# HKUST-Aerial-Robotics/DenseSurfelMapping

Hardware: AMD Instinct MI355X
Metric: depth frames fused/sec @ KITTI 1226x370 (higher is better)
Workload: dtype f32

## Files before the change

densesurfelmapping_amd/csrc/dsm_k_superpixel.h:

```cpp
#pragma once
#include "dsm_k_common.h"

namespace dsm {

constexpr int kInitLanes = 16, kInitSeedsPerBlock = 256 / kInitLanes;
template <bool BATCH> __global__ __launch_bounds__(256) void k_init_seeds(const DeviceCtx ctx, const DeviceCtx *__restrict__ batch) {
    const BlockOf blk = block_of<BATCH>();
    DeviceCtx batch_ctx;
    if (BATCH) batch_ctx = load_ctx(batch + blk.z);
    const DeviceCtx *__restrict__ c = BATCH ? &batch_ctx : &ctx;
    const int tid = threadIdx.x, lane = lane_id();
    const int r = tid & (kInitLanes - 1);
    const int s = blk.x * kInitSeedsPerBlock + tid / kInitLanes;
    if (blk.x == 0 && tid < kSweeps * kWorkers) c->first_empty[tid] = kIntMax;
    if (blk.x == 0 && tid == 0) c->work_count[0] = c->fit_big_count[0] = 0;
    if (blk.x == 0 && tid < 2 * kSweeps) c->rest_count[tid] = 0;
    const FrameParams &fp = c->params[(unsigned)(c->cursor[0] * c->cursor_mul + c->cursor_add) % (unsigned)c->n_params];
    const uint8_t *img = c->img_base + (int64_t)fp.slot * c->slot_elems;
    const float *dep = c->depth_base + (int64_t)fp.slot * c->slot_elems;
    if (blk.x == 0 && tid < 64) {
        FrameCur *wc = c->cur;
        const int t = tid;
        if (t < 16) wc->p.pose[t] = fp.pose[t];
        else if (t < 32) wc->p.inv[t - 16] = fp.inv[t - 16];
        else if (t == 32) { wc->p.ref_idx = fp.ref_idx; wc->p.slot = fp.slot; }
        else if (t == 33) wc->img = img;
        else if (t == 34) wc->dep = dep;
    }
    const int w = c->w, h = c->h, pitch = c->pitch;
    const bool live = s < c->n_seed;
    const int sc = live ? s : 0;
    const int gx = sc % c->gw, gy = sc / c->gw;
    int ix = gx * kCell + kCell / 2, iy = gy * kCell + kCell / 2;
    if (ix > w - 1) ix = w - 1;
    if (iy > h - 1) iy = h - 1;
    const int wx0 = gx * kCell + kCell / 2 - kCell, wy0 = gy * kCell + kCell / 2 - kCell;
    const int x_lo = wx0 < 0 ? 0 : wx0, x_hi = wx0 + 2 * kCell > w - 1 ? w - 1 : wx0 + 2 * kCell;
    const int y_lo = wy0 < 0 ? 0 : wy0, y_hi = wy0 + 2 * kCell > h - 1 ? h - 1 : wy0 + 2 * kCell;
    const int y = wy0 + r;
    const bool row_in = y >= y_lo && y < y_hi;
    float md = dep[iy * pitch + ix];
    const float mi = (float)img[iy * pitch + ix];
    float4 v[4];
#pragma unroll
    for (int q = 0; q < 4; q++) {
        const int x = wx0 + 4 * q;
        v[q] = (row_in && x >= 0) ? *reinterpret_cast<const float4 *>(dep + y * pitch + x) : make_float4(0, 0, 0, 0);
    }
    bool hit = false;
    float first = 0.0f;
#pragma unroll
    for (int q = 3; q >= 0; q--) {
        const float e[4] = {v[q].x, v[q].y, v[q].z, v[q].w};
#pragma unroll
        for (int t = 3; t >= 0; t--) {
            const int x = wx0 + 4 * q + t;
            if (row_in && x >= x_lo && x < x_hi && e[t] > flt_below(0.01)) { hit = true; first = e[t]; }
        }
    }
    const unsigned long long m = __ballot(hit);
    const unsigned rows = (unsigned)(m >> (lane & ~(kInitLanes - 1))) & 0xffffu;
    const int src = (lane & ~(kInitLanes - 1)) + (rows ? __ffs((int)rows) - 1 : 0);
    const float scanned = __shfl(first, src);
    if (md < flt_above(0.01) && rows) md = scanned;
    if (!live || r != 0) return;
    c->core[s] = make_float4((float)ix, (float)iy, mi, md);
    c->inv_depth[s] = 1.0 / (double)md;
    c->tmin[s] = -1;
}

template <bool BATCH> __global__ __launch_bounds__(256) void k_init_seeds_lanes(const DeviceCtx ctx, const DeviceCtx *__restrict__ batch) {
    const BlockOf blk = block_of<BATCH>();
    DeviceCtx batch_ctx;
    if (BATCH) batch_ctx = load_ctx(batch + blk.z);
    const DeviceCtx *__restrict__ c = BATCH ? &batch_ctx : &ctx;
    const int tid = threadIdx.x;
    const int s = blk.x * 256 + tid;
    if (blk.x == 0 && tid < kSweeps * kWorkers) c->first_empty[tid] = kIntMax;
    if (blk.x == 0 && tid == 0) c->work_count[0] = c->fit_big_count[0] = 0;
    if (blk.x == 0 && tid < 2 * kSweeps) c->rest_count[tid] = 0;
    const FrameParams &fp = c->params[(unsigned)(c->cursor[0] * c->cursor_mul + c->cursor_add) % (unsigned)c->n_params];
    const uint8_t *img = c->img_base + (int64_t)fp.slot * c->slot_elems;
    const float *dep = c->depth_base + (int64_t)fp.slot * c->slot_elems;
    if (blk.x == 0 && tid < 64) {
        FrameCur *wc = c->cur;
        const int t = tid;
        if (t < 16) wc->p.pose[t] = fp.pose[t];
        else if (t < 32) wc->p.inv[t - 16] = fp.inv[t - 16];
        else if (t == 32) { wc->p.ref_idx = fp.ref_idx; wc->p.slot = fp.slot; }
        else if (t == 33) wc->img = img;
        else if (t == 34) wc->dep = dep;
    }
    const int w = c->w, h = c->h, pitch = c->pitch;
    const bool live = s < c->n_seed;
    const int sc = live ? s : 0;
    int gx, gy;
    seed_cell(c, sc, gx, gy);
    int ix = gx * kCell + kCell / 2, iy = gy * kCell + kCell / 2;
    if (ix > w - 1) ix = w - 1;
    if (iy > h - 1) iy = h - 1;
    float md = dep[iy * pitch + ix];
    const float mi = (float)img[iy * pitch + ix];
    const bool need = live && md < flt_above(0.01);
    if (__ballot(need) != 0) {
        const int wx0 = gx * kCell + kCell / 2 - kCell, wy0 = gy * kCell + kCell / 2 - kCell;
        const int x_lo = wx0 < 0 ? 0 : wx0, x_hi = wx0 + 2 * kCell > w - 1 ? w - 1 : wx0 + 2 * kCell;
        const int y_lo = wy0 < 0 ? 0 : wy0, y_hi = wy0 + 2 * kCell > h - 1 ? h - 1 : wy0 + 2 * kCell;
        bool pending = need;
#pragma unroll 1
        for (int r0 = 0; r0 < 2 * kCell && __ballot(pending) != 0; r0 += 2) {
            float4 v[2][4];
            bool row_in[2];
#pragma unroll
            for (int k = 0; k < 2; k++) {
                const int y = wy0 + r0 + k;
                row_in[k] = pending && y >= y_lo && y < y_hi;
#pragma unroll
                for (int q = 0; q < 4; q++) {
                    const int x = wx0 + 4 * q;
                    v[k][q] = (row_in[k] && x >= 0) ? *reinterpret_cast<const float4 *>(dep + y * pitch + x) : make_float4(0, 0, 0, 0);
                }
            }
#pragma unroll
            for (int k = 0; k < 2; k++) {
                bool hit = false;
                float first = 0.0f;
#pragma unroll
                for (int q = 3; q >= 0; q--) {
                    const float e[4] = {v[k][q].x, v[k][q].y, v[k][q].z, v[k][q].w};
#pragma unroll
                    for (int t = 3; t >= 0; t--) {
                        const int x = wx0 + 4 * q + t;
                        if (row_in[k] && x >= x_lo && x < x_hi && e[t] > flt_below(0.01)) { hit = true; first = e[t]; }
                    }
                }
                if (pending && hit) { md = first; pending = false; }
            }
        }
    }
    if (!live) return;
    c->core[s] = make_float4((float)ix, (float)iy, mi, md);
    c->inv_depth[s] = 1.0 / (double)md;
    c->tmin[s] = -1;
}

constexpr int kTileW = 64, kTileCellsX = kTileW / kCell + 2;
template <int COLS> struct AssignTile {
    static constexpr int kH = 4 * COLS, kCellsY = (kH + kCell - 1) / kCell + 2;
};

constexpr int kResolveHeld = 8;
__device__ void resolve_worklist(const DeviceCtx *c, label_t *label) {
    const int n = c->work_count[0];
    if (n == 0) return;
    const int tid = threadIdx.x;
    int p[kResolveHeld], l[kResolveHeld], pk[kResolveHeld];
    bool ev[kResolveHeld];
#pragma unroll
    for (int k = 0; k < kResolveHeld; k++) p[k] = tid + k * 256 < n ? c->worklist[tid + k * 256] : -1;
#pragma unroll
    for (int k = 0; k < kResolveHeld; k++) {
        l[k] = p[k] >= 0 ? (int)label[p[k]] : 0;
        pk[k] = p[k] >= 0 ? (int)c->cand[p[k]] : 0;
    }
    for (;;) {
        int changed = 0;
        int tl[kResolveHeld], tp[kResolveHeld];
#pragma unroll
        for (int k = 0; k < kResolveHeld; k++) {
            if (k * 256 >= n) break;
            tl[k] = load_coherent(&c->tmin[l[k]]);
            tp[k] = load_coherent(&c->tmin[pk[k]]);
        }
#pragma unroll
        for (int k = 0; k < kResolveHeld; k++) {
            ev[k] = k * 256 < n && p[k] >= 0 && tl[k] < p[k];
            if (ev[k] && tp[k] > p[k]) {
                atomicMin(&c->tmin[pk[k]], p[k]);
                changed = 1;
            }
        }
        for (int i = tid + kResolveHeld * 256; i < n; i += 256) {
            const int q = c->worklist[i];
            const int lq = label[q], pq = c->cand[q];
            if (load_coherent(&c->tmin[lq]) < q && load_coherent(&c->tmin[pq]) > q) {
                atomicMin(&c->tmin[pq], q);
                changed = 1;
            }
        }
        if (!__syncthreads_or(changed)) break;
    }
#pragma unroll
    for (int k = 0; k < kResolveHeld; k++)
        if (ev[k]) label[p[k]] = (label_t)pk[k];
    for (int i = tid + kResolveHeld * 256; i < n; i += 256) {
        const int q = c->worklist[i];
        const int lq = label[q];
        if (load_coherent(&c->tmin[lq]) < q) label[q] = c->cand[q];
    }
}

template <bool FIRST, bool BATCH, int COLS> __global__ __launch_bounds__(256) void k_assign(const DeviceCtx ctx, const DeviceCtx *__restrict__ batch, int sweep) {
    constexpr int kColumn = COLS, kTileH = AssignTile<COLS>::kH, kTileCellsY = AssignTile<COLS>::kCellsY;
    const BlockOf blk = block_of<BATCH>();
    DeviceCtx batch_ctx;
    if (BATCH) batch_ctx = load_ctx(batch + blk.z);
    const DeviceCtx *__restrict__ c = BATCH ? &batch_ctx : &ctx;
    constexpr int kCells = kTileCellsX * kTileCellsY;
    __shared__ float4 s_core[kCells];
    __shared__ double s_inv[kCells];
    __shared__ float s_f[5][kCells];
    __shared__ unsigned short s_open[kTileW * kTileH];
    __shared__ int s_n_open;
    const FrameParams &fp = frame_params(c);
    const uint8_t *img = frame_image(c, fp);
    const float *dep = frame_depth(c, fp);
    const label_t *label_in = c->label;
    const int w = c->w, h = c->h, pitch = c->pitch, gw = c->gw, gh = c->gh;
    const int bx = blk.x * kTileW, by = blk.y * kTileH;
    const int cx0 = bx / kCell - 1, cy0 = by / kCell - 1;
    const int tid = threadIdx.x;
    if (tid == 0) s_n_open = 0;
    if (tid < kCells) {
        int gx = cx0 + tid % kTileCellsX, gy = cy0 + tid / kTileCellsX;
        gx = gx < 0 ? 0 : (gx > gw - 1 ? gw - 1 : gx);
        gy = gy < 0 ? 0 : (gy > gh - 1 ? gh - 1 : gy);
        const float4 v = c->core[gy * gw + gx];
        const double inv = c->inv_depth[gy * gw + gx];
        s_core[tid] = v;
        s_inv[tid] = inv;
        s_f[0][tid] = v.x * 0.25f;
        s_f[1][tid] = v.y * 0.25f;
        s_f[2][tid] = v.z;
        s_f[3][tid] = seed_s20(v.w, inv);
        s_f[4][tid] = v.w;
    }
    __syncthreads();
    auto settle = [&](int p, int l, int pick, int tl, int tp) {
        if (pick < 0) {
            atomicOr(c->status, kStatusBadPick);
            if (FIRST) label_put(c->label, (unsigned)p, 0);
        } else if (FIRST) {
            label_put(c->label, (unsigned)p, pick);
        } else if (tl == -1) {
            if (pick != l) label_put(c->label, (unsigned)p, pick);
            if (tp > p) atomicMin(&c->tmin[pick], p);
        } else if (pick != l) {
            label_put(c->cand, (unsigned)p, pick);
            const unsigned long long m = __ballot(true);
            const int rk = rank_below(m);
            int base = 0;
            if (rk == 0) base = atomicAdd(c->work_count, __popcll(m));
            base = __builtin_amdgcn_readlane(base, __ffsll((long long)m) - 1);
            c->worklist[base + rk] = p;
        }
    };
    auto tmin_of = [&](int s) {
        return __hip_atomic_load(reinterpret_cast<const int32_t *>(reinterpret_cast<const char *>(c->tmin) + ((unsigned)s << 2)), __ATOMIC_RELAXED,
                                 __HIP_MEMORY_SCOPE_AGENT);
    };
    const int x = bx + (tid & (kTileW - 1)), y0 = by + (tid / kTileW) * kColumn;
    if (x < w && y0 < h) {
        float pix_i[kColumn], pix_d[kColumn];
        int lab[kColumn], tl[kColumn], pick[kColumn];
        bool live[kColumn], sure[kColumn];
        const unsigned p0 = (unsigned)(__mul24(y0, pitch) + x);
#pragma unroll
        for (int r = 0; r < kColumn; r++) {
            const unsigned p = y0 + r < h ? p0 + (unsigned)(r * pitch) : p0, p4 = p << 2;
            pix_i[r] = (float)ld_off(img, p);
            pix_d[r] = ld_off(dep, p4);
            lab[r] = FIRST ? 0 : (int)ld_off(label_in, p << 1);
        }
        if (!FIRST) {
            const unsigned s_last = (unsigned)c->n_seed - 1u;
#pragma unroll
            for (int r = 0; r < kColumn; r++) tl[r] = ld_off(c->tmin, ((unsigned)lab[r] < s_last ? (unsigned)lab[r] : s_last) << 2);
        }
        const int li0 = __mul24(((y0 >> 3) - ((y0 & 7) < 4 ? 1 : 0)) - cy0, kTileCellsX) + (((x >> 3) - ((x & 7) < 4 ? 1 : 0)) - cx0);
        const PickCol quad = pick_col(x, y0, gw, gh, [&](int k, int, int, float &sx4, float &sy4, float &si, float &sd, float &s20) {
            const int li = li0 + (k >> 1) + (k & 1) * kTileCellsX;
            sx4 = s_f[0][li]; sy4 = s_f[1][li]; si = s_f[2][li]; s20 = s_f[3][li]; sd = s_f[4][li];
        });
#pragma unroll
        for (int r = 0; r < kColumn; r++) {
            const int y = y0 + r;
            live[r] = y < h && has_candidate_cell(x, y, gw, gh);
            const FastPick fpk = pick_seed_fast(quad, y, pix_i[r], pix_d[r], gw);
            pick[r] = fpk.seed;
            sure[r] = fpk.sure;
            if (FIRST && y < h && !live[r]) label_put(c->label, p0 + (unsigned)(r * pitch), -1);
        }
#pragma unroll
        for (int r = 0; r < kColumn; r++) {
            const bool open = live[r] && !sure[r];
            const unsigned long long m = __ballot(open);
            if (m) {
                const int rk = rank_below(m);
                int base = 0;
                if (open && rk == 0) base = atomicAdd(&s_n_open, __popcll(m));
                base = __builtin_amdgcn_readlane(base, __ffsll((long long)m) - 1);
                if (open) s_open[base + rk] = (unsigned short)((((tid / kTileW) * kColumn + r) << 6) | (tid & (kTileW - 1)));
            }
            live[r] = live[r] && !open;
        }
        int tp[kColumn];
        if (!FIRST) {
#pragma unroll
            for (int r = 0; r < kColumn; r++) tp[r] = tmin_of(live[r] ? pick[r] : 0);
        }
#pragma unroll
        for (int r = 0; r < kColumn; r++)
            if (live[r]) settle((int)p0 + r * pitch, lab[r], pick[r], FIRST ? 0 : tl[r], FIRST ? 0 : tp[r]);
    }
    __syncthreads();
    const int n_open = s_n_open;
    for (int i = tid; i < n_open; i += 256) {
        const unsigned e = s_open[i];
        const int ox = bx + (int)(e & 63u), oy = by + (int)(e >> 6);
        const unsigned p = (unsigned)(__mul24(oy, pitch) + ox);
        const float pi = (float)ld_off(img, p), pd = ld_off(dep, p << 2);
        const int l = FIRST ? 0 : label_at(label_in, p);
        const int pick = pick_seed(ox, oy, pi, pd, gw, gh, [&](int gx, int gy, float &sx, float &sy, float &si, bool &has_d, double &inv_d) {
            const int li = __mul24(gy - cy0, kTileCellsX) + (gx - cx0);
            const float4 v = s_core[li];
            sx = v.x; sy = v.y; si = v.z;
            has_d = v.w > 0;
            inv_d = s_inv[li];
        });
        settle((int)p, l, pick, FIRST ? 0 : ld_off(c->tmin, (unsigned)l << 2), FIRST || pick < 0 ? 0 : tmin_of(pick));
    }
}

template <bool BATCH> __global__ __launch_bounds__(256) void k_resolve(const DeviceCtx ctx, const DeviceCtx *__restrict__ batch, int sweep) {
    const BlockOf blk = block_of<BATCH>();
    DeviceCtx batch_ctx;
    if (BATCH) batch_ctx = load_ctx(batch + blk.z);
    const DeviceCtx *__restrict__ c = BATCH ? &batch_ctx : &ctx;
    resolve_worklist(c, c->label);
}

__device__ __forceinline__ float huber_ordered_sum(const float *lt, int nd, const unsigned long long tail[4],
                                                   const unsigned long long pos[4], double hr) {
    float a = 0.0f;
#pragma unroll
    for (int k = 0; k < 4; k++) {
        const int lim = nd - k * 64 < 64 ? nd - k * 64 : 64;
        if (lim <= 0) break;
        for (int j = 0; j < lim; j += kBlk) {
            const Blk16 v = load_blk(lt + k * 64 + j);
            const unsigned t16 = (unsigned)(tail[k] >> j) & 0xffffu, p16 = (unsigned)(pos[k] >> j) & 0xffffu;
            if (t16 == 0) {
#pragma unroll
                for (int q = 0; q < kBlk; q++) a += v.e[q];
            } else {
#pragma unroll
                for (int q = 0; q < kBlk; q++) {
                    const float a_core = a + v.e[q];
                    const float a_tail = (float)((double)a + (((p16 >> q) & 1u) ? hr : -1 * hr));
                    a = ((t16 >> q) & 1u) ? a_tail : a_core;
                }
            }
        }
    }
    return a;
}

__device__ __forceinline__ float huber_passes_wave(const float *dl, float *lt, int nd, float md, int it0, double hr, int lane) {
    const float hr_above = flt_above(hr);
    float dk[4];
#pragma unroll
    for (int k = 0; k < 4; k++) dk[k] = (k * 64 + lane < nd) ? dl[k * 64 + lane] : 0.0f;
    const int nk = (nd + 63) >> 6;
    for (int it = it0; it < 5; it++) {
        unsigned long long tail[4] = {0, 0, 0, 0}, pos[4] = {0, 0, 0, 0};
        int n_core = 0;
#pragma unroll
        for (int k = 0; k < 4; k++) {
            if (k >= nk) break;
            const int idx = k * 64 + lane;
            const bool valid = idx < nd;
            const float r = md - dk[k];
            const bool core = valid && fabsf(r) < hr_above;
            if (valid) lt[idx] = 2 * r;
            tail[k] = __ballot(valid && !core);
            pos[k] = __ballot(valid && !core && r > 0);
            n_core += __popcll(__ballot(core));
        }
        wave_lds_sync();
        const float a = huber_ordered_sum(lt, nd, tail, pos, hr);
        const float b = (float)(2 * n_core);
        const float delta = huber_newton_step(a, b);
        md = md + delta;
        wave_lds_sync();
        if (fabsf(delta) < flt_above(0.01)) break;
    }
    return md;
}

constexpr int kWin = 2 * kCell;

__device__ __forceinline__ void update_seed_finish(const DeviceCtx *__restrict__ c, int sweep, int s, int lane, int wx0, int wy0,
                                                   const float4 old, float *dl, float *lt, int cnt, int sdx, int sdy, int si, int nd) {
    stamp(c, sweep, s, 2, lane);
    const int cnt_si = wave_sum(si | (cnt << 16));
    cnt = cnt_si >> 16;
    si = cnt_si & 0xffff;
    if (cnt == 0) {
        if (lane == 0) atomicMin(&c->first_empty[sweep * kWorkers + chunk_of(c->n_seed, s)], s);
        return;
    }
    const int packed = wave_sum(sdx | (sdy << 16));
    const int sx = (packed & 0xffff) + cnt * wx0, sy = (packed >> 16) + cnt * wy0;
    wave_lds_sync();
    const float fn = (float)cnt;
    const float mi = (float)si / fn, mx = (float)sx / fn, my = (float)sy / fn;
    const float moved = fabsf(old.z - mi) + fabsf(old.x - mx) + fabsf(old.y - my);
    const int stable = moved < flt_above(0.2) ? 1 : 0;
    stamp(c, sweep, s, 3, lane);
    float md = 0.0f;
    wave_priority(nd);
    if (nd > 0) {
        pad_column(dl, nd, lane);
        pad_column(lt, nd, lane);
        wave_lds_sync();
        md = ordered_sum(dl, nd) / (float)nd;
        stamp(c, sweep, s, 4, lane);
        if (!mean_depth_is_settled(md)) md = huber_passes_wave(dl, lt, nd, md, 0, c->huber, lane);
    }
    stamp(c, sweep, s, 5, lane);
    if (kWaveStamps && c->stamps && lane == 0) c->stamps[((int64_t)sweep * c->n_seed + s) * 8 + 7] = nd;
    if (lane == 0) {
        c->core_stage[s] = make_float4(mx, my, mi, md);
        c->stable_stage[s] = stable;
    }
}

__device__ __forceinline__ void update_seed_wave(const DeviceCtx *__restrict__ c, int sweep, int s, float *dl, float *lt) {
    const int lane = lane_id();
    stamp(c, sweep, s, 0, lane);
    const FrameParams &fp = frame_params(c);
    const uint8_t *img = frame_image(c, fp);
    const float *dep = frame_depth(c, fp);
    const label_t *lbl = c->label;
    const int w = c->w, h = c->h, pitch = c->pitch;
    int gx, gy;
    seed_cell(c, s, gx, gy);
    const int wx0 = gx * kCell + kCell / 2 - kCell, wy0 = gy * kCell + kCell / 2 - kCell;
    const int t_self = c->tmin[s];
    if (t_self == kIntMax) return;
    const float4 old = c->core[s];
    stamp(c, sweep, s, 1, lane);
    int cnt = 0, sdx = 0, sdy = 0, si = 0, nd = 0;
    int lab[4], pi[4];
    float pd[4];
    bool pimg[4];
    const int x = wx0 + (lane & (kWin - 1)), y0 = wy0 + (lane >> 4);
    const bool x_in = x >= 0 && x < w;
    const int key0 = __mul24(y0, pitch) + x, row4 = 4 * pitch;
#pragma unroll
    for (int k = 0; k < 4; k++) {
        const int y = y0 + 4 * k;
        pimg[k] = x_in && y >= 0 && y < h;
        const int pk = pimg[k] ? key0 + k * row4 : 0;
        const unsigned o4 = (unsigned)pk << 2;
        lab[k] = (int)ld_off(lbl, (unsigned)pk << 1);
        pd[k] = ld_off(dep, o4);
        pi[k] = (int)ld_off(img, (unsigned)pk);
    }
#pragma unroll
    for (int k = 0; k < 4; k++) {
        const int idx = k * 64 + lane;
        const int y = y0 + 4 * k;
        const bool mem = pimg[k] && x < w - 1 && y < h - 1 && lab[k] == s;
        const float d = mem ? pd[k] : 0.0f;
        if (mem) {
            cnt += 1; sdx += idx & (kWin - 1); sdy += idx >> 4; si += pi[k];
        }
        const bool dv = mem && d > flt_below(0.1);
        const unsigned long long m = __ballot(dv);
        if (dv) dl[nd + rank_below(m)] = d;
        nd += __popcll(m);
    }
// ... 307 lines not shown
```

densesurfelmapping_amd/csrc/dsm_kernels.hip:

```cpp
#include "dsm_device.h"

#include "dsm_k_common.h"
#include "dsm_k_superpixel.h"
#include "dsm_k_planes.h"
#include "dsm_k_map.h"
#include "dsm_k_cloud.h"
#include "dsm_k_mesh.h"
#include "dsm_k_render.h"
#include "dsm_k_grid.h"
#include "dsm_k_field.h"
#include "dsm_k_carve.h"
#include "dsm_k_align.h"

namespace dsm {

const char *const kStageNames[kNumStages] = {
    "init_seeds", "assign_0",  "update_seeds_0", "commit_seeds_0", "assign_1",    "resolve_1",    "update_seeds_1", "commit_seeds_1",
    "assign_2",   "resolve_2", "update_seeds_2", "commit_seeds_2", "seed_points", "seed_fit", "fuse_surfels", "frame_tail",
};

template <bool E33>
static hipError_t launch_frame_as(const DeviceCtx &hc, int map_upper_bound, int tail_map_bound, bool with_compaction,
                                  hipStream_t st, hipEvent_t *ev, int stage_lo, int stage_hi, const DeviceCtx *d_batch, int n_batch, int lanes_from) {
    int stage = 0;
    hipError_t err = hipSuccess;
    const bool batched = d_batch != nullptr;
    const unsigned nz = batched ? (unsigned)n_batch : 1u;
#define hipLaunchStage(kernel_single, kernel_batch, grid, block, ...)                                        \
    do {                                                                                                     \
        if (stage - 1 >= stage_lo && stage - 1 <= stage_hi) {                                                \
            const dim3 g_((grid).x, (grid).y, nz);                                                           \
            if (batched) hipLaunchKernelGGL(kernel_batch, g_, block, 0, st, hc, d_batch, ##__VA_ARGS__);   \
            else hipLaunchKernelGGL(kernel_single, g_, block, 0, st, hc, d_batch, ##__VA_ARGS__);          \
        }                                                                                                    \
    } while (0)
#define DSM_MARK()                                                                      \
    do {                                                                                \
        if (ev) {                                                                       \
            err = hipEventRecord(ev[stage], st);                                        \
            if (err != hipSuccess) return err;                                          \
        }                                                                               \
        stage++;                                                                        \
    } while (0)
    const int S = hc.n_seed;
    const dim3 g_seed_thr((S + 255) / 256);
    const dim3 g_seed_wave((S + 3) / 4);
    const dim3 g_seed_lane((S + 63) / 64);
    const dim3 g_seed_rest((S + 63) / 64 + kRestOverBlocks);
    const bool lanes = batched && n_batch >= (lanes_from > 0 ? lanes_from : kLaneBatch);
    const dim3 g_tile1((hc.w + kTileW - 1) / kTileW, (hc.h + AssignTile<1>::kH - 1) / AssignTile<1>::kH);
    const dim3 g_tile4((hc.w + kTileW - 1) / kTileW, (hc.h + AssignTile<4>::kH - 1) / AssignTile<4>::kH);
    if (ev) hipLaunchKernelGGL(k_delay, dim3(1), dim3(64), 0, st, 40000LL);
    DSM_MARK();
    if (lanes) hipLaunchStage(k_init_seeds_lanes<true>, k_init_seeds_lanes<true>, g_seed_thr, dim3(256));
    else hipLaunchStage(k_init_seeds<false>, k_init_seeds<true>, dim3((S + kInitSeedsPerBlock - 1) / kInitSeedsPerBlock), dim3(256));
    DSM_MARK();
    for (int sweep = 0; sweep < kSweeps; sweep++) {
        if (sweep == 0) {
            if (lanes) hipLaunchStage((k_assign<true, true, 4>), (k_assign<true, true, 4>), g_tile4, dim3(256), sweep);
            else hipLaunchStage((k_assign<true, false, 1>), (k_assign<true, true, 1>), g_tile1, dim3(256), sweep);
            DSM_MARK();
        } else {
            if (lanes) hipLaunchStage((k_assign<false, true, 4>), (k_assign<false, true, 4>), g_tile4, dim3(256), sweep);
            else hipLaunchStage((k_assign<false, false, 1>), (k_assign<false, true, 1>), g_tile1, dim3(256), sweep);
            DSM_MARK();
            hipLaunchStage(k_resolve<false>, k_resolve<true>, dim3(1), dim3(256), sweep);
            DSM_MARK();
        }
        if (lanes) {
            hipLaunchStage(k_update_seeds<true>, k_update_seeds<true>, g_seed_lane, dim3(64), sweep);
            hipLaunchStage(k_update_seeds_rest<true>, k_update_seeds_rest<true>, g_seed_rest, dim3(64), sweep);
        } else {
            hipLaunchStage(k_update_seeds_wave<false>, k_update_seeds_wave<true>, g_seed_wave, dim3(256), sweep);
        }
        DSM_MARK();
        hipLaunchStage(k_commit_seeds<false>, k_commit_seeds<true>, g_seed_thr, dim3(256), sweep);
        DSM_MARK();
    }
    if (lanes) {
        hipLaunchStage(k_pixel_normals<true>, k_pixel_normals<true>, dim3((hc.w + 63) / 64, (hc.h + 4 * kNormalRows - 1) / (4 * kNormalRows)), dim3(256));
        hipLaunchStage(k_seed_stats<true>, k_seed_stats<true>, g_seed_lane, dim3(64));
    } else {
        hipLaunchStage(k_seed_points<false>, k_seed_points<true>, g_seed_wave, dim3(256));
    }
    DSM_MARK();
    const int fit_masks = lanes ? 1 : 0;
    hipLaunchStage((k_seed_fit<false, kFitAll>), (k_seed_fit<true, kFitSmall>), dim3((S + kFitSeeds - 1) / kFitSeeds), dim3(64), fit_masks);
    if (batched) hipLaunchStage((k_seed_fit<false, kFitAll>), (k_seed_fit<true, kFitLarge>), dim3(kFitLargeBlocks), dim3(64), fit_masks);
    hipLaunchStage((k_seed_finish<false, E33>), (k_seed_finish<true, E33>), g_seed_thr, dim3(256));
    DSM_MARK();
    int fuse_blocks = (map_upper_bound + 255) / 256;
    if (fuse_blocks < 1) fuse_blocks = 1;
    const int fuse_cap = batched ? resident_blocks(k_fuse_surfels<true, E33>, 256, kFuseBlocksPerCu) : resident_blocks(k_fuse_surfels<false, E33>, 256, kFuseBlocksPerCu);
    if (fuse_blocks > fuse_cap) fuse_blocks = fuse_cap;
    if (batched && nz > 1 && fuse_blocks > (fuse_cap / nz > 1 ? fuse_cap / nz : 1)) fuse_blocks = fuse_cap / nz > 1 ? fuse_cap / nz : 1;
    hipLaunchStage((k_fuse_surfels<false, E33>), (k_fuse_surfels<true, E33>), dim3(fuse_blocks), dim3(256));
    DSM_MARK();
    int tail_blocks = 1;
    if (with_compaction && tail_map_bound > kTailFastWords * 64) {
        tail_blocks = 1 + (tail_map_bound / 64 + kTailChunkWords) / kTailChunkWords;
        if (tail_blocks > kTailMaxBlocks) tail_blocks = kTailMaxBlocks;
    }
    hipLaunchStage(k_frame_tail<false>, k_frame_tail<true>, dim3(tail_blocks), dim3(1024), with_compaction ? 1 : 0);
    DSM_MARK();
    if (ev) {
        err = hipEventRecord(ev[stage], st);
        if (err != hipSuccess) return err;
    }
#undef DSM_MARK
#undef hipLaunchStage
    return hipGetLastError();
}

hipError_t launch_frame(const DeviceCtx &hc, bool eigen33, int map_upper_bound, int tail_map_bound, bool with_compaction,
                        hipStream_t st, hipEvent_t *ev, int stage_lo, int stage_hi, const DeviceCtx *d_batch, int n_batch, int lanes_from) {
    return eigen33 ? launch_frame_as<true>(hc, map_upper_bound, tail_map_bound, with_compaction, st, ev, stage_lo, stage_hi, d_batch, n_batch, lanes_from)
                   : launch_frame_as<false>(hc, map_upper_bound, tail_map_bound, with_compaction, st, ev, stage_lo, stage_hi, d_batch, n_batch, lanes_from);
}

}
```

densesurfelmapping_amd/csrc/dsm_math.h:

```cpp
#pragma once
#include <math.h>
#include <stdint.h>

#if defined(__HIPCC__) || defined(__HIP__)
#define DSM_HD __host__ __device__ __forceinline__
#else
#define DSM_HD static inline
#endif

namespace dsm {

constexpr int kCell = 8;
constexpr int kSweeps = 3;
constexpr int kWorkers = 10;
constexpr double kAngleCos = 0.1;

struct Intrinsics {
    float fx, fy, cx, cy;
};

DSM_HD constexpr float flt_below(double c) {
    const float f = (float)c;
    return (double)f <= c ? f : __builtin_bit_cast(float, __builtin_bit_cast(uint32_t, f) - 1u);
}
// ... 16 lines not shown
    float cost = 0.0f;
    cost += dist / (float)((kCell / 2) * (kCell / 2));
    float di = si - pix_i;
    cost = (float)((double)cost + div_by_100((double)(di * di)));
    no_d = cost;
    with_d = cost;
    if (seed_has_depth && pix_invd > 0) {
        float dd = (float)(seed_inv_depth - (double)pix_invd);
        with_d = (float)((double)cost + (double)(dd * dd) * 400.0);
        return true;
    }
    return false;
}

DSM_HD float pixel_inv_depth(float d) {
    float invd = 0.0f;
    if (d > flt_below(0.01)) invd = 1.0f / d;
    return invd;
}

DSM_HD bool has_candidate_cell(int x, int y, int gw, int gh) { return x < gw * kCell + kCell / 2 && y < gh * kCell + kCell / 2; }

template <typename LoadSeed>
DSM_HD int pick_seed(int x, int y, float pix_i, float pix_d, int gw, int gh, LoadSeed load) {
    const float invd = pixel_inv_depth(pix_d);
    const int bx = x / kCell, by = y / kCell;
    float best_d = 1e6f, best_n = 1e6f;
    int arg_d = -1, arg_n = -1;
    bool all_depth = true;
    const int xr = x % kCell, yr = y % kCell;
    const int gx0 = bx - (xr < kCell / 2 ? 1 : 0), gy0 = by - (yr < kCell / 2 ? 1 : 0);
    for (int jx = 0; jx < 2; jx++) {
        const int gx = gx0 + jx;
        if (!(gx >= 0 && gx < gw) || (jx == 1 && xr == kCell / 2)) continue;
        for (int jy = 0; jy < 2; jy++) {
            const int gy = gy0 + jy;
            if (!(gy >= 0 && gy < gh) || (jy == 1 && yr == kCell / 2)) continue;
            const int s = gy * gw + gx;
            float sx, sy, si;
            bool has_d;
            double inv_d;
            load(gx, gy, sx, sy, si, has_d, inv_d);
            float cn, cd;
            const bool with = pixel_cost(sx, sy, si, has_d, inv_d, pix_i, invd, x, y, cn, cd);
            all_depth = all_depth && with;
            if (cd < best_d) { best_d = cd; arg_d = s; }
            if (cn < best_n) { best_n = cn; arg_n = s; }
        }
    }
    return all_depth ? arg_d : arg_n;
}

struct FastCost {
    float c, err;
};
constexpr float kFastU = 5.9604645e-8f;

#if defined(__HIP_DEVICE_COMPILE__)
typedef float f32x2 __attribute__((ext_vector_type(2)));
DSM_HD f32x2 f2_make(float a, float b) { f32x2 r; r.x = a; r.y = b; return r; }
DSM_HD f32x2 f2_fma(f32x2 a, f32x2 b, f32x2 c) { return __builtin_elementwise_fma(a, b, c); }
DSM_HD f32x2 f2_mul(f32x2 a, f32x2 b) { return a * b; }
DSM_HD f32x2 f2_sub(f32x2 a, f32x2 b) { return a - b; }
DSM_HD float rcp_1ulp(float d) { return __builtin_amdgcn_rcpf(d); }
#else
struct f32x2 {
    float x, y;
};
DSM_HD f32x2 f2_make(float a, float b) { return f32x2{a, b}; }
DSM_HD f32x2 f2_fma(f32x2 a, f32x2 b, f32x2 c) { return f32x2{__builtin_fmaf(a.x, b.x, c.x), __builtin_fmaf(a.y, b.y, c.y)}; }
DSM_HD f32x2 f2_mul(f32x2 a, f32x2 b) { return f32x2{a.x * b.x, a.y * b.y}; }
DSM_HD f32x2 f2_sub(f32x2 a, f32x2 b) { return f32x2{a.x - b.x, a.y - b.y}; }
DSM_HD float rcp_1ulp(float d) {
    const float q = 1.0f / d;
    uint32_t b = __builtin_bit_cast(uint32_t, q);
    if ((b & 0x7f800000u) == 0u) return 0.0f;
    uint32_t hsh = __builtin_bit_cast(uint32_t, d) * 2654435761u;
    hsh ^= hsh >> 15;
    const uint32_t k = hsh % 3u;
    if (q == q && (b & 0x7f800000u) != 0x7f800000u) b += k == 1u ? 1u : (k == 2u ? 0xffffffffu : 0u);
    return __builtin_bit_cast(float, b);
}
#endif
DSM_HD f32x2 f2_splat(float a) { return f2_make(a, a); }

DSM_HD bool pixel_has_inv_depth(float d) { return d > flt_below(0.01) && d < __builtin_inff(); }
DSM_HD float pixel_p20(float d) { return 20.0f * rcp_1ulp(d); }
DSM_HD float seed_s20(float mean_depth, double inv_depth) { return mean_depth > 0 ? (float)(20.0 * inv_depth) : 0.0f; }

DSM_HD float fast_cost_df(float s20_abs_max) { return __builtin_fmaf(12.0f * kFastU, s20_abs_max, 2e-36f); }
DSM_HD float fast_cost_slack(float ad20, float df) {
    const float e2 = __builtin_fmaf(16.0f * kFastU, ad20, df);
    return e2 * __builtin_fmaf(2.0f, ad20, e2);
}
DSM_HD float fast_cost_err(float c, float slack) { return __builtin_fmaf(20.0f * kFastU, c, slack); }

DSM_HD FastCost pixel_cost_fast(float sx, float sy, float si, float s20, bool with_depth, float pix_i, float p20, int x, int y) {
    const float ddx = sx - (float)x;
    const float ax16 = (ddx * ddx) * 0.0625f;
    const float ddyq = sy * 0.25f - (float)y * 0.25f;
    const float dist16 = __builtin_fmaf(ddyq, ddyq, ax16);
    const float t = (si - pix_i) * 0.1f;
    const float c_no = __builtin_fmaf(t, t, dist16);
    const float dd20 = __builtin_fmaf(s20, with_depth ? 1.0f : 0.0f, with_depth ? -p20 : 0.0f);
    FastCost r;
    r.c = __builtin_fmaf(dd20, dd20, c_no);
    r.err = fast_cost_err(r.c, fast_cost_slack(fabsf(dd20), fast_cost_df(fabsf(s20))));
    return r;
}

struct PickCol {
    f32x2 ax16[2];
    f32x2 ax16_edge[2];
    f32x2 sy4[2], si[2], s20[2];
    bool depth_ok[2];
    float df;
    int base;
};
constexpr float kPickPenalty = 1e30f;
template <typename LoadSeedF> DSM_HD PickCol pick_col(int x, int y, int gw, int gh, LoadSeedF load) {
    PickCol q;
    const int xr = x & (kCell - 1), yr = y & (kCell - 1);
    const int gx0 = (x >> 3) - (xr < kCell / 2 ? 1 : 0), gy0 = (y >> 3) - (yr < kCell / 2 ? 1 : 0);
    static_assert(kCell == 8, "the shifts above");
    q.base = gy0 * gw + gx0;
    const bool col_ok[2] = {gx0 >= 0, gx0 + 1 < gw && xr != kCell / 2};
    const bool row_in[2] = {gy0 >= 0, gy0 + 1 < gh};
    float sx4[4], sy4[4], si[4], sd[4], s20[4];
    for (int k = 0; k < 4; k++) load(k, gx0 + (k >> 1), gy0 + (k & 1), sx4[k], sy4[k], si[k], sd[k], s20[k]);
    const f32x2 xq = f2_splat((float)x * 0.25f);
    for (int j = 0; j < 2; j++) {
        const f32x2 ddx4 = f2_sub(f2_make(sx4[2 * j], sx4[2 * j + 1]), xq);
        const f32x2 a = f2_mul(ddx4, ddx4);
        const bool in0 = col_ok[j] && row_in[0], in1 = col_ok[j] && row_in[1];
        q.ax16[j] = f2_make(in0 ? a.x : kPickPenalty, in1 ? a.y : kPickPenalty);
        q.ax16_edge[j] = f2_make(in0 ? a.x : kPickPenalty, kPickPenalty);
        q.sy4[j] = f2_make(sy4[2 * j], sy4[2 * j + 1]);
        q.si[j] = f2_make(si[2 * j], si[2 * j + 1]);
        q.s20[j] = f2_make(s20[2 * j], s20[2 * j + 1]);
    }
    q.df = fast_cost_df(fmaxf(fmaxf(fabsf(s20[0]), fabsf(s20[1])), fmaxf(fabsf(s20[2]), fabsf(s20[3]))));
    for (int j = 0; j < 2; j++)
        q.depth_ok[j] = !row_in[j] | ((!col_ok[0] | (sd[j] > 0)) & (!col_ok[1] | (sd[2 + j] > 0)));
    return q;
}
struct FastPickTrace {
    float err;
    bool all_depth;
};
struct FastPick {
    int seed;
    bool sure;
};
DSM_HD FastPick pick_seed_fast(const PickCol &q, int y, float pix_i, float pix_d, int gw, FastPickTrace *trace = nullptr) {
    const bool edge = (y & (kCell - 1)) == kCell / 2;
    const bool all_depth = pixel_has_inv_depth(pix_d) && q.depth_ok[0] && (q.depth_ok[1] || edge);
    const f32x2 mm = f2_splat(all_depth ? 1.0f : 0.0f), p20m = f2_splat(all_depth ? -pixel_p20(pix_d) : 0.0f);
    const f32x2 yq = f2_splat((float)y * 0.25f), pi = f2_splat(pix_i), tenth = f2_splat(0.1f);
    f32x2 c[2], dd20[2];
    for (int j = 0; j < 2; j++) {
        const f32x2 ddyq = f2_sub(q.sy4[j], yq);
        const f32x2 dist16 = f2_fma(ddyq, ddyq, edge ? q.ax16_edge[j] : q.ax16[j]);
        const f32x2 t = f2_mul(f2_sub(q.si[j], pi), tenth);
        const f32x2 c_no = f2_fma(t, t, dist16);
        dd20[j] = f2_fma(q.s20[j], mm, p20m);
        c[j] = f2_fma(dd20[j], dd20[j], c_no);
    }
    const float ck[4] = {c[0].x, c[0].y, c[1].x, c[1].y};
    const float ad_max = fmaxf(fmaxf(fabsf(dd20[0].x), fabsf(dd20[0].y)), fmaxf(fabsf(dd20[1].x), fabsf(dd20[1].y)));
    uint32_t key[4];
    for (int k = 0; k < 4; k++) key[k] = (__builtin_bit_cast(uint32_t, ck[k]) & ~3u) | (uint32_t)k;
    const uint32_t lo01 = key[0] < key[1] ? key[0] : key[1], hi01 = key[0] < key[1] ? key[1] : key[0];
    const uint32_t lo23 = key[2] < key[3] ? key[2] : key[3], hi23 = key[2] < key[3] ? key[3] : key[2];
    const uint32_t first = lo01 < lo23 ? lo01 : lo23;
    const uint32_t mid_a = lo01 < lo23 ? lo23 : lo01, mid_b = hi01 < hi23 ? hi01 : hi23;
    const uint32_t second = mid_a < mid_b ? mid_a : mid_b;
    const float c1 = __builtin_bit_cast(float, first), c2 = fminf(__builtin_bit_cast(float, second), 2e6f);
    const float err = fast_cost_err(c2, fast_cost_slack(ad_max, q.df));
    if (trace) { trace->err = err; trace->all_depth = all_depth; }
    FastPick r;
    r.seed = q.base + (int)(first & 1u) * gw + (int)((first >> 1) & 1u);
    r.sure = c1 + err < c2 - err && c1 + err < 1e6f;
    return r;
}
template <typename LoadSeedF>
DSM_HD FastPick pick_seed_fast(int x, int y, float pix_i, float pix_d, int gw, int gh, LoadSeedF load, FastPickTrace *trace = nullptr) {
    return pick_seed_fast(pick_col(x, y, gw, gh, load), y, pix_i, pix_d, gw, trace);
}

DSM_HD float huber_newton_step(float a, float b) { return (-a) / (b + 10.0f); }

DSM_HD bool mean_depth_is_settled(float md) { return md == __builtin_inff(); }

DSM_HD float huber_mean_depth(const float *list, int n, float sum, double huber) {
    const float hr_above = flt_above(huber);
    float md = sum / (float)n;
    if (mean_depth_is_settled(md)) return md;
    for (int it = 0; it < 5; it++) {
        float a = 0, b = 0;
        for (int k = 0; k < n; k++) {
            float r = md - list[k];
            if (fabsf(r) < hr_above) {
                a += 2 * r;
                b += 2;
            } else {
                a = (float)((double)a + (r > 0 ? huber : -1 * huber));
            }
        }
        float delta = huber_newton_step(a, b);
        md = md + delta;
        if (fabsf(delta) < flt_above(0.01)) break;
    }
    return md;
}

struct WindowPixel {
    bool member, has_depth, inlier;
};
DSM_HD WindowPixel window_pixel(bool row_in, bool col_in, bool label_is_seed, float d, float mean_depth, float hr_above) {
    WindowPixel p;
    p.member = row_in && col_in && label_is_seed;
    p.has_depth = p.member && d > flt_below(0.05);
    p.inlier = p.has_depth && fabsf(mean_depth - d) < hr_above;
    return p;
}

DSM_HD void back_project(const Intrinsics &k, float u, float v, float d, float &x, float &y, float &z) {
    x = (u - k.cx) / k.fx * d;
    y = (v - k.cy) / k.fy * d;
    z = d;
}

DSM_HD float ray_coeff(int u, float c, float f) { return ((float)u - c) / f; }

DSM_HD bool pixel_normal_rays(float rx0, float rx1, float ry0, float ry1, float d, float d_right, float d_down, float &nx, float &ny,
                              float &nz) {
    constexpr float kMin = flt_above(0.1);
    if (d < kMin || d_right < kMin || d_down < kMin) return false;
    const float px = rx0 * d, py = ry0 * d, pz = d;
    float rx = rx1 * d_right, ry = ry0 * d_right, rz = d_right;
    float dx = rx0 * d_down, dy = ry1 * d_down, dz = d_down;
    rx = rx - px; ry = ry - py; rz = rz - pz;
    dx = dx - px; dy = dy - py; dz = dz - pz;
    float ax = ry * dz - rz * dy, ay = rz * dx - rx * dz, az = rx * dy - ry * dx;
    float len = sqrtf(ax * ax + ay * ay + az * az);
    ax /= len; ay /= len; az /= len;
    float va = (ax * px + ay * py + az * pz) / sqrtf(px * px + py * py + pz * pz);
    if (fabsf(va) < flt_above(kAngleCos)) return false;
    nx = ax; ny = ay; nz = az;
    return true;
}

DSM_HD bool pixel_normal(const Intrinsics &k, int x, int y, float d, float d_right, float d_down, float &nx,
                         float &ny, float &nz) {
    constexpr float kMin = flt_above(0.1);
    if (d < kMin || d_right < kMin || d_down < kMin) return false;
    float px, py, pz, rx, ry, rz, dx, dy, dz;
    back_project(k, (float)x, (float)y, d, px, py, pz);
    back_project(k, (float)(x + 1), (float)y, d_right, rx, ry, rz);
    back_project(k, (float)x, (float)(y + 1), d_down, dx, dy, dz);
    rx = rx - px; ry = ry - py; rz = rz - pz;
    dx = dx - px; dy = dy - py; dz = dz - pz;
    float ax = ry * dz - rz * dy, ay = rz * dx - rx * dz, az = rx * dy - ry * dx;
    float len = sqrtf(ax * ax + ay * ay + az * az);
    ax /= len; ay /= len; az /= len;
    float va = (ax * px + ay * py + az * pz) / sqrtf(px * px + py * py + pz * pz);
    if (fabsf(va) < flt_above(kAngleCos)) return false;
    nx = ax; ny = ay; nz = az;
    return true;
}

template <typename T> DSM_HD void inverse4(const T *a, T *o) {
    T s0 = a[0] * a[5] - a[1] * a[4], s1 = a[0] * a[9] - a[1] * a[8], s2 = a[0] * a[13] - a[1] * a[12];
    T s3 = a[4] * a[9] - a[5] * a[8], s4 = a[4] * a[13] - a[5] * a[12], s5 = a[8] * a[13] - a[9] * a[12];
    T c5 = a[10] * a[15] - a[11] * a[14], c4 = a[6] * a[15] - a[7] * a[14], c3 = a[6] * a[11] - a[7] * a[10];
    T c2 = a[2] * a[15] - a[3] * a[14], c1 = a[2] * a[11] - a[3] * a[10], c0 = a[2] * a[7] - a[3] * a[6];
    T det = s0 * c5 - s1 * c4 + s2 * c3 + s3 * c2 - s4 * c1 + s5 * c0;
    T id = (T)1 / det;
    o[0] = (a[5] * c5 - a[9] * c4 + a[13] * c3) * id;
    o[4] = (-a[4] * c5 + a[8] * c4 - a[12] * c3) * id;
    o[8] = (a[7] * s5 - a[11] * s4 + a[15] * s3) * id;
    o[12] = (-a[6] * s5 + a[10] * s4 - a[14] * s3) * id;
    o[1] = (-a[1] * c5 + a[9] * c2 - a[13] * c1) * id;
    o[5] = (a[0] * c5 - a[8] * c2 + a[12] * c1) * id;
    o[9] = (-a[3] * s5 + a[11] * s2 - a[15] * s1) * id;
    o[13] = (a[2] * s5 - a[10] * s2 + a[14] * s1) * id;
    o[2] = (a[1] * c4 - a[5] * c2 + a[13] * c0) * id;
    o[6] = (-a[0] * c4 + a[4] * c2 - a[12] * c0) * id;
    o[10] = (a[3] * s4 - a[7] * s2 + a[15] * s0) * id;
    o[14] = (-a[2] * s4 + a[6] * s2 - a[14] * s0) * id;
    o[3] = (-a[1] * c3 + a[5] * c1 - a[9] * c0) * id;
    o[7] = (a[0] * c3 - a[4] * c1 + a[8] * c0) * id;
    o[11] = (-a[3] * s3 + a[7] * s1 - a[11] * s0) * id;
    o[15] = (a[2] * s3 - a[6] * s1 + a[10] * s0) * id;
}

struct Inv4Tables {
    signed char det2[12][4];
    signed char det_terms[6][3];
    signed char out[16][7];
};
constexpr Inv4Tables kInv4 = {
    {{0, 5, 1, 4}, {0, 9, 1, 8}, {0, 13, 1, 12}, {4, 9, 5, 8}, {4, 13, 5, 12}, {8, 13, 9, 12},
     {2, 7, 3, 6}, {2, 11, 3, 10}, {2, 15, 3, 14}, {6, 11, 7, 10}, {6, 15, 7, 14}, {10, 15, 11, 14}},
    {{0, 11, 1}, {1, 10, -1}, {2, 9, 1}, {3, 8, 1}, {4, 7, -1}, {5, 6, 1}},
    {{5, 11, 9, 10, 13, 9, 1},
     {1, 11, 9, 8, 13, 7, -1},
     {1, 10, 5, 8, 13, 6, 1},
     {1, 9, 5, 7, 9, 6, -1},
     {4, 11, 8, 10, 12, 9, -1},
     {0, 11, 8, 8, 12, 7, 1},
     {0, 10, 4, 8, 12, 6, -1},
     {0, 9, 4, 7, 8, 6, 1},
     {7, 5, 11, 4, 15, 3, 1},
     {3, 5, 11, 2, 15, 1, -1},
     {3, 4, 7, 2, 15, 0, 1},
     {3, 3, 7, 1, 11, 0, -1},
     {6, 5, 10, 4, 14, 3, -1},
     {2, 5, 10, 2, 14, 1, 1},
     {2, 4, 6, 2, 14, 0, -1},
     {2, 3, 6, 1, 10, 0, 1}},
};
template <typename T> DSM_HD T inv4_det2(const T *a, int t) {
    return a[kInv4.det2[t][0]] * a[kInv4.det2[t][1]] - a[kInv4.det2[t][2]] * a[kInv4.det2[t][3]];
}
template <typename T> DSM_HD T inv4_det(const T *D) {
    T det = D[kInv4.det_terms[0][0]] * D[kInv4.det_terms[0][1]];
    for (int i = 1; i < 6; i++) {
        const T prod = D[kInv4.det_terms[i][0]] * D[kInv4.det_terms[i][1]];
        det = kInv4.det_terms[i][2] > 0 ? det + prod : det - prod;
    }
    return det;
}
template <typename T> DSM_HD T inv4_entry(const T *a, const T *D, T inv_det, int k) {
    const signed char *e = kInv4.out[k];
    const T g = (T)e[6];
// ... 417 lines not shown
```

Measured before the change: 47790.

## Cache per-pixel depth terms and skip tmin atomics in quiet assign tiles

The first assign sweep now computes a per-pixel depth term (has-inverse-depth flag folded into p20) and stores it in the normals buffer, so later sweeps reload it instead of recomputing from raw depth. A separate fill kernel covers the case where the run starts after the first sweep. Tiles whose neighbouring seeds are all stable (tmin == -1) take a plain path that skips the per-pixel tmin atomic loads and writes labels directly. This reuses the normals buffer as scratch, which assumes it is not live during the assign sweeps, and adds a ballot plus extra branching.

```diff
diff --git a/densesurfelmapping_amd/csrc/dsm_k_superpixel.h b/densesurfelmapping_amd/csrc/dsm_k_superpixel.h
--- a/densesurfelmapping_amd/csrc/dsm_k_superpixel.h
+++ b/densesurfelmapping_amd/csrc/dsm_k_superpixel.h
@@ -149,6 +149,19 @@
     static constexpr int kH = 4 * COLS, kCellsY = (kH + kCell - 1) / kCell + 2;
 };
 
+__device__ __forceinline__ float *pixel_terms(const DeviceCtx *c) { return c->normals; }
+template <bool BATCH> __global__ __launch_bounds__(256) void k_fill_pixel_terms(const DeviceCtx ctx, const DeviceCtx *__restrict__ batch) {
+    const BlockOf blk = block_of<BATCH>();
+    DeviceCtx batch_ctx;
+    if (BATCH) batch_ctx = load_ctx(batch + blk.z);
+    const DeviceCtx *__restrict__ c = BATCH ? &batch_ctx : &ctx;
+    const float *dep = frame_depth(c, frame_params(c));
+    const int x = blk.x * 256 + (int)threadIdx.x, y = blk.y;
+    if (x >= c->w || y >= c->h) return;
+    const unsigned p4 = (unsigned)(__mul24(y, c->pitch) + x) << 2;
+    st_off(pixel_terms(c), p4, pixel_term(ld_off(dep, p4)));
+}
+
 constexpr int kResolveHeld = 8;
 __device__ void resolve_worklist(const DeviceCtx *c, label_t *label) {
     const int n = c->work_count[0];
@@ -211,22 +224,25 @@
     __shared__ double s_inv[kCells];
     __shared__ float s_f[5][kCells];
     __shared__ unsigned short s_open[kTileW * kTileH];
-    __shared__ int s_n_open;
+    __shared__ int s_n_open, s_quiet;
     const FrameParams &fp = frame_params(c);
     const uint8_t *img = frame_image(c, fp);
     const float *dep = frame_depth(c, fp);
     const label_t *label_in = c->label;
+    float *term = pixel_terms(c);
     const int w = c->w, h = c->h, pitch = c->pitch, gw = c->gw, gh = c->gh;
     const int bx = blk.x * kTileW, by = blk.y * kTileH;
     const int cx0 = bx / kCell - 1, cy0 = by / kCell - 1;
     const int tid = threadIdx.x;
     if (tid == 0) s_n_open = 0;
+    bool cell_unstable = true;
     if (tid < kCells) {
         int gx = cx0 + tid % kTileCellsX, gy = cy0 + tid / kTileCellsX;
         gx = gx < 0 ? 0 : (gx > gw - 1 ? gw - 1 : gx);
         gy = gy < 0 ? 0 : (gy > gh - 1 ? gh - 1 : gy);
         const float4 v = c->core[gy * gw + gx];
         const double inv = c->inv_depth[gy * gw + gx];
+        if (!FIRST) cell_unstable = c->tmin[gy * gw + gx] == -1;
         s_core[tid] = v;
         s_inv[tid] = inv;
         s_f[0][tid] = v.x * 0.25f;
@@ -235,7 +251,13 @@
         s_f[3][tid] = seed_s20(v.w, inv);
         s_f[4][tid] = v.w;
     }
+    static_assert(kCells <= 64, "the staging threads are one wave");
+    if (!FIRST && tid < 64) {
+        const bool all = __ballot(!cell_unstable) == 0;
+        if (tid == 0) s_quiet = all ? 1 : 0;
+    }
     __syncthreads();
+    const bool quiet = !FIRST && __builtin_amdgcn_readfirstlane(s_quiet) != 0;
     auto settle = [&](int p, int l, int pick, int tl, int tp) {
         if (pick < 0) {
             atomicOr(c->status, kStatusBadPick);
@@ -261,16 +283,25 @@
     };
     const int x = bx + (tid & (kTileW - 1)), y0 = by + (tid / kTileW) * kColumn;
     if (x < w && y0 < h) {
-        float pix_i[kColumn], pix_d[kColumn];
+        float pix_i[kColumn], pix_t[kColumn];
         int lab[kColumn], tl[kColumn], pick[kColumn];
         bool live[kColumn], sure[kColumn];
         const unsigned p0 = (unsigned)(__mul24(y0, pitch) + x);
+        unsigned p4[kColumn];
 #pragma unroll
         for (int r = 0; r < kColumn; r++) {
-            const unsigned p = y0 + r < h ? p0 + (unsigned)(r * pitch) : p0, p4 = p << 2;
+            const unsigned p = y0 + r < h ? p0 + (unsigned)(r * pitch) : p0;
+            p4[r] = p << 2;
             pix_i[r] = (float)ld_off(img, p);
-            pix_d[r] = ld_off(dep, p4);
+            pix_t[r] = ld_off(FIRST ? dep : term, p4[r]);
             lab[r] = FIRST ? 0 : (int)ld_off(label_in, p << 1);
+        }
+        if (FIRST) {
+#pragma unroll
+            for (int r = 0; r < kColumn; r++) {
+                pix_t[r] = pixel_term(pix_t[r]);
+                st_off(term, p4[r], pix_t[r]);
+            }
         }
         if (!FIRST) {
             const unsigned s_last = (unsigned)c->n_seed - 1u;
@@ -286,7 +317,7 @@
         for (int r = 0; r < kColumn; r++) {
             const int y = y0 + r;
             live[r] = y < h && has_candidate_cell(x, y, gw, gh);
-            const FastPick fpk = pick_seed_fast(quad, y, pix_i[r], pix_d[r], gw);
+            const FastPick fpk = pick_seed_fast_terms(quad, y, pix_i[r], term_has_inv_depth(pix_t[r]), pix_t[r], gw);
             pick[r] = fpk.seed;
             sure[r] = fpk.sure;
             if (FIRST && y < h && !live[r]) label_put(c->label, p0 + (unsigned)(r * pitch), -1);
@@ -305,13 +336,30 @@
             live[r] = live[r] && !open;
         }
         int tp[kColumn];
+        bool plain = false;
         if (!FIRST) {
-#pragma unroll
-            for (int r = 0; r < kColumn; r++) tp[r] = tmin_of(live[r] ? pick[r] : 0);
-        }
-#pragma unroll
-        for (int r = 0; r < kColumn; r++)
-            if (live[r]) settle((int)p0 + r * pitch, lab[r], pick[r], FIRST ? 0 : tl[r], FIRST ? 0 : tp[r]);
+            bool trip = !quiet;
+#pragma unroll
+            for (int r = 0; r < kColumn; r++) trip = trip || tl[r] != -1;
+#pragma unroll
+            for (int r = 0; r < kColumn; r++) tp[r] = -1;
+            if (trip) {
+#pragma unroll
+                for (int r = 0; r < kColumn; r++) tp[r] = tmin_of(live[r] ? pick[r] : 0);
+            }
+            plain = !trip;
+#pragma unroll
+            for (int r = 0; r < kColumn; r++) plain = plain && (!live[r] || pick[r] >= 0);
+        }
+        if (!FIRST && __ballot(!plain) == 0) {
+#pragma unroll
+            for (int r = 0; r < kColumn; r++)
+                if (live[r] && pick[r] != lab[r]) st_off(c->label, p4[r] >> 1, (label_t)pick[r]);
+        } else {
+#pragma unroll
+            for (int r = 0; r < kColumn; r++)
+                if (live[r]) settle((int)p0 + r * pitch, lab[r], pick[r], FIRST ? 0 : tl[r], FIRST ? 0 : tp[r]);
+        }
     }
     __syncthreads();
     const int n_open = s_n_open;
@@ -328,7 +376,8 @@
             has_d = v.w > 0;
             inv_d = s_inv[li];
         });
-        settle((int)p, l, pick, FIRST ? 0 : ld_off(c->tmin, (unsigned)l << 2), FIRST || pick < 0 ? 0 : tmin_of(pick));
+        const int tl = FIRST ? 0 : ld_off(c->tmin, (unsigned)l << 2);
+        settle((int)p, l, pick, tl, FIRST || pick < 0 ? 0 : (quiet && tl == -1 ? -1 : tmin_of(pick)));
     }
 }
 
diff --git a/densesurfelmapping_amd/csrc/dsm_kernels.hip b/densesurfelmapping_amd/csrc/dsm_kernels.hip
--- a/densesurfelmapping_amd/csrc/dsm_kernels.hip
+++ b/densesurfelmapping_amd/csrc/dsm_kernels.hip
@@ -55,6 +55,12 @@
     if (lanes) hipLaunchStage(k_init_seeds_lanes<true>, k_init_seeds_lanes<true>, g_seed_thr, dim3(256));
     else hipLaunchStage(k_init_seeds<false>, k_init_seeds<true>, dim3((S + kInitSeedsPerBlock - 1) / kInitSeedsPerBlock), dim3(256));
     DSM_MARK();
+    constexpr int kStageAssign0 = 1, kStageAssign1 = 4, kStageAssign2 = 8;
+    if (stage_lo > kStageAssign0 && stage_lo <= kStageAssign2 && stage_hi >= (stage_lo <= kStageAssign1 ? kStageAssign1 : kStageAssign2)) {
+        const dim3 g_fill((hc.w + 255) / 256, hc.h, nz);
+        if (batched) hipLaunchKernelGGL(k_fill_pixel_terms<true>, g_fill, dim3(256), 0, st, hc, d_batch);
+        else hipLaunchKernelGGL(k_fill_pixel_terms<false>, g_fill, dim3(256), 0, st, hc, d_batch);
+    }
     for (int sweep = 0; sweep < kSweeps; sweep++) {
         if (sweep == 0) {
             if (lanes) hipLaunchStage((k_assign<true, true, 4>), (k_assign<true, true, 4>), g_tile4, dim3(256), sweep);
diff --git a/densesurfelmapping_amd/csrc/dsm_math.h b/densesurfelmapping_amd/csrc/dsm_math.h
--- a/densesurfelmapping_amd/csrc/dsm_math.h
+++ b/densesurfelmapping_amd/csrc/dsm_math.h
@@ -192,10 +192,13 @@
     int seed;
     bool sure;
 };
-DSM_HD FastPick pick_seed_fast(const PickCol &q, int y, float pix_i, float pix_d, int gw, FastPickTrace *trace = nullptr) {
+DSM_HD float pixel_term(float d) { return pixel_has_inv_depth(d) ? pixel_p20(d) : -1.0f; }
+DSM_HD bool term_has_inv_depth(float t) { return t >= 0.0f; }
+
+DSM_HD FastPick pick_seed_fast_terms(const PickCol &q, int y, float pix_i, bool has, float p20, int gw, FastPickTrace *trace = nullptr) {
     const bool edge = (y & (kCell - 1)) == kCell / 2;
-    const bool all_depth = pixel_has_inv_depth(pix_d) && q.depth_ok[0] && (q.depth_ok[1] || edge);
-    const f32x2 mm = f2_splat(all_depth ? 1.0f : 0.0f), p20m = f2_splat(all_depth ? -pixel_p20(pix_d) : 0.0f);
+    const bool all_depth = has && q.depth_ok[0] && (q.depth_ok[1] || edge);
+    const f32x2 mm = f2_splat(all_depth ? 1.0f : 0.0f), p20m = f2_splat(all_depth ? -p20 : 0.0f);
     const f32x2 yq = f2_splat((float)y * 0.25f), pi = f2_splat(pix_i), tenth = f2_splat(0.1f);
     f32x2 c[2], dd20[2];
     for (int j = 0; j < 2; j++) {
@@ -222,6 +225,9 @@
     r.seed = q.base + (int)(first & 1u) * gw + (int)((first >> 1) & 1u);
     r.sure = c1 + err < c2 - err && c1 + err < 1e6f;
     return r;
+}
+DSM_HD FastPick pick_seed_fast(const PickCol &q, int y, float pix_i, float pix_d, int gw, FastPickTrace *trace = nullptr) {
+    return pick_seed_fast_terms(q, y, pix_i, pixel_has_inv_depth(pix_d), pixel_p20(pix_d), gw, trace);
 }
 template <typename LoadSeedF>
 DSM_HD FastPick pick_seed_fast(int x, int y, float pix_i, float pix_d, int gw, int gh, LoadSeedF load, FastPickTrace *trace = nullptr) {
```

After: 47420. No clear change (-0.8%).
